# Streampunk/phaneron

Measured on AMD Instinct MI355X. Metric: frames/sec, 4-layer 2160p50 composite pipeline (v210 unpack->CSC->combine->CSC->v210 pack), higher is better.
Workload: dtype f32

## Files before the change

phaneron_amd/csrc/ph_kernels_lds.hip:

```cpp
#include "ph_device.h"
#include "ph_kernels.h"
#include "ph_ldslut.h"

#include <atomic>
#include <cstdlib>

#include <type_traits>

#pragma clang fp contract(off)

#ifndef PH_PROBE
#define PH_PROBE 0
#endif
#if PH_PROBE
constexpr int kProbeWords = 16;
__device__ unsigned long long g_fused_probe[2048 * kProbeWords];
extern "C" int ph_debug_fused_probe(unsigned long long *out, int n_words) {
  return (int)hipMemcpyFromSymbol(out, HIP_SYMBOL(g_fused_probe), (size_t)n_words * 8);
}
#define PH_STAMP_ENTRY() \
  const unsigned long long ph_entry_cycles = __builtin_amdgcn_s_memtime(), ph_entry_ticks = __builtin_amdgcn_s_memrealtime()
#define PH_STAMP(k) PH_STAMP_IF(k, tile_begin == wg_begin)
#define PH_STAMP_IF(k, first_tile)                                                   \
  do {                                                                               \
    if (threadIdx.x == 0 && (first_tile)) {                                          \
      g_fused_probe[blockIdx.x * kProbeWords + 2 * (k)] = __builtin_amdgcn_s_memtime();       \
      g_fused_probe[blockIdx.x * kProbeWords + 2 * (k) + 1] = __builtin_amdgcn_s_memrealtime(); \
      if ((k) == 0) {                                                                \
        g_fused_probe[blockIdx.x * kProbeWords + 10] = ph_entry_cycles;              \
        g_fused_probe[blockIdx.x * kProbeWords + 11] = ph_entry_ticks;               \
      }                                                                              \
    }                                                                                \
  } while (0)
#else
#define PH_STAMP_ENTRY() do { } while (0)
#define PH_STAMP(k) do { } while (0)
#define PH_STAMP_IF(k, first_tile) do { } while (0)
#endif

#ifndef PH_BALANCE_WAVES
#define PH_BALANCE_WAVES 1
#endif
#if PH_BALANCE_WAVES
__device__ __forceinline__ void ph_set_wave_priority(int level) {
  switch (level) {
    case 3: __builtin_amdgcn_s_setprio(3); break;
    case 2: __builtin_amdgcn_s_setprio(2); break;
    case 1: __builtin_amdgcn_s_setprio(1); break;
    default: __builtin_amdgcn_s_setprio(0); break;
  }
}
#define PH_BALANCE(p) ph_set_wave_priority(3 - ((p) * 4) / P)
#else
#define PH_BALANCE(p) do { } while (0)
#endif

namespace ph {


__device__ __forceinline__ uint4 write_quad_lds(const float (&rgb)[18], const WriteK &wk, const LutK &lut) {
  uint32_t y[6], u[3], v[3];
#pragma unroll
  for (int j = 0; j < 6; ++j) {
    if ((j & 1) == 0) {
      const Yuv1 c = write_px_lds(rgb[3 * j], rgb[3 * j + 1], rgb[3 * j + 2], wk, lut);
      y[j] = c.y, u[j >> 1] = c.u, v[j >> 1] = c.v;
    } else {
      y[j] = write_px_luma_lds(rgb[3 * j], rgb[3 * j + 1], rgb[3 * j + 2], wk, lut);
    }
  }
  return pack_quad(y, u, v);
}

#ifndef PH_FUSED_SPLIT
#define PH_FUSED_SPLIT 0
#endif
typedef uint32_t fused_head_line __attribute__((ext_vector_type(16)));
struct FusedHead {
  fused_head_line l0, l1, l2;
  __device__ __forceinline__ uint32_t word(int byte) const { return byte < 64 ? l0[byte / 4] : byte < 128 ? l1[byte / 4 - 16] : l2[byte / 4 - 32]; }
  template <typename P>
  __device__ __forceinline__ P ptr(int byte) const { return (P)((uintptr_t)word(byte) | ((uintptr_t)word(byte + 4) << 32)); }
  __device__ __forceinline__ LutK lut_k(int byte) const {
    return LutK{__uint_as_float(word(byte)), __uint_as_float(word(byte + 4)), __uint_as_float(word(byte + 8)), __uint_as_float(word(byte + 12)), word(byte + 16)};
  }
};
typedef const __attribute__((address_space(1))) ph_u4v *global_quad_ptr;
typedef const __attribute__((address_space(1))) uint32_t *global_u32_ptr;
typedef const __attribute__((address_space(4))) float *const_f32_ptr;
__device__ __forceinline__ uint4 load_stream(global_quad_ptr p) {
  const ph_u4v v = __builtin_nontemporal_load(p);
  return make_uint4(v.x, v.y, v.z, v.w);
}
__device__ __forceinline__ ReadK load_read_k(const_f32_ptr cm, const_f32_ptr gm) {
  ReadK k;
  k.r = make_float4(cm[0], cm[1], cm[2], cm[3]);
  k.g = make_float4(cm[4], cm[5], cm[6], cm[7]);
  k.b = make_float4(cm[8], cm[9], cm[10], cm[11]);
#pragma unroll
  for (int i = 0; i < 9; ++i) k.gm[i] = gm[i];
  return k;
}
__device__ __forceinline__ WriteK load_write_k(const_f32_ptr cm) {
  WriteK k;
  k.y = make_float4(cm[0], cm[1], cm[2], cm[3]);
  k.u = make_float4(cm[4], cm[5], cm[6], cm[7]);
  k.v = make_float4(cm[8], cm[9], cm[10], cm[11]);
  return k;
}
static_assert(kFusedHeadBytes == 3 * sizeof(fused_head_line), "fused_head_load asks for three lines");
__device__ __forceinline__ FusedHead fused_head_load() {
  FusedHead h;
  const auto *args = __builtin_amdgcn_kernarg_segment_ptr();
  asm volatile("s_load_dwordx16 %0, %3, 0x0\n\ts_load_dwordx16 %1, %3, 0x40\n\ts_load_dwordx16 %2, %3, 0x80\n\ts_waitcnt lgkmcnt(0)"
               : "=&s"(h.l0), "=&s"(h.l1), "=&s"(h.l2)
               : "s"(args));
  return h;
}

template <int N, int P, int BS, bool PIPE = false, int MODE = 0, bool TAIL = false>
__global__ __launch_bounds__(BS) void fused_v210_combine_lds_kernel(FusedLdsArgs a, uint32_t *handoff = nullptr) {
  static_assert(!TAIL || (!PIPE && MODE == 0), "the tail instantiation exists for the shipped form only");
  PH_STAMP_ENTRY();
  const FusedHead head = fused_head_load();
  const uint32_t total_quads = head.word(offsetof(FusedLdsArgs, total_quads)), wg_per_job = head.word(offsetof(FusedLdsArgs, wg_per_job));
  const uint32_t per_wg = head.word(offsetof(FusedLdsArgs, per_wg));
  uint32_t job = fused_job_of(blockIdx.x, head.word(offsetof(FusedLdsArgs, magic_wg)));
  asm("" : "+s"(job));
  const uint32_t wg_in_job = blockIdx.x - job * wg_per_job;
  auto layer_ptr = [&](int l) { return reinterpret_cast<const uint4 *>(job ? a.more_layers[job - 1][l] : a.layers[l]); };
  const uint32_t wg_begin = wg_in_job * per_wg;
  const uint32_t wg_end = wg_begin + per_wg < total_quads ? wg_begin + per_wg : total_quads;
  if (wg_begin >= wg_end) return;
  const uint32_t tile_quads = BS * P;
  auto quad_at = [&](uint32_t tile_begin, int p) {
    const uint32_t f = tile_begin + p * BS + threadIdx.x;
    return f < wg_end ? f : wg_end - 1;
  };
  uint4 w;
  if (job) w = load_stream(layer_ptr(0) + quad_at(wg_begin, 0));
  else w = load_stream(head.ptr<global_quad_ptr>(offsetof(FusedLdsArgs, layers)) + quad_at(wg_begin, 0));
  const uint32_t *const rd_blob = (const uint32_t *)head.ptr<global_u32_ptr>(offsetof(FusedLdsArgs, rd_blob));
  const uint32_t rd_bytes = head.word(offsetof(FusedLdsArgs, rd_bytes)), rd_hole = head.word(offsetof(FusedLdsArgs, rd_hole));
  PH_STAMP_IF(0, true);
  if (MODE != 2) lds_lut_load<BS, false>(rd_blob, rd_bytes, rd_hole);
  __builtin_amdgcn_sched_barrier(0);
  const ReadK rk = load_read_k(head.ptr<const_f32_ptr>(offsetof(FusedLdsArgs, rd_cm)), head.ptr<const_f32_ptr>(offsetof(FusedLdsArgs, rd_gm)));
  const WriteK wk = load_write_k(head.ptr<const_f32_ptr>(offsetof(FusedLdsArgs, wr_cm)));
  LutK rlut = head.lut_k(offsetof(FusedLdsArgs, rd_k)), wlut = head.lut_k(offsetof(FusedLdsArgs, wr_k));
  asm("" : "+v"(rlut.a_base), "+v"(rlut.delta_base), "+v"(wlut.a_base), "+v"(wlut.delta_base));
  const uint32_t *const wr_blob = (const uint32_t *)head.ptr<global_u32_ptr>(offsetof(FusedLdsArgs, wr_blob));
  const uint32_t wr_bytes = head.word(offsetof(FusedLdsArgs, wr_bytes)), wr_hole = head.word(offsetof(FusedLdsArgs, wr_hole));
  uint4 *const out_ptr = reinterpret_cast<uint4 *>(job ? a.more_out[job - 1] : a.out);
  const bool std_matrix = ycbcr_matrix_is_standard(rk);
  for (uint32_t tile_begin = wg_begin; tile_begin < wg_end; tile_begin += tile_quads) {
    uint32_t st[P][9];
    auto quad_of = [&](int p) { return quad_at(tile_begin, p); };
    if (tile_begin != wg_begin) {
      w = load_stream(layer_ptr(0) + quad_of(0));
      if (MODE == 0) lds_lut_load<BS, false>(rd_blob, rd_bytes, rd_hole);
    }
    auto slot_kind = [&](uint32_t f) -> uint32_t {
      const uint32_t g = f - __umulhi(f, a.magic_qpp) * a.quads_per_line_pitch;
      return g < a.quads_per_line_used ? 0u : (g == a.quads_per_line_used && a.tail_px) ? 1u : 2u;
    };
    auto phase1_slice = [&](auto tag, uint4 w, uint32_t f, uint32_t f_next, bool more, uint32_t(&st)[9]) -> uint4 {
      const bool in_tail = TAIL && slot_kind(f) == 1u;
      const float last = TAIL ? (in_tail ? 0.0f : 1.0f) : 1.0f;
      float acc[18];
#pragma unroll
      for (int i = 0; i < 18; ++i) acc[i] = 0.0f;
#pragma unroll 1
      for (int l = 0; l < N; ++l) {
        uint4 nxt = w;
        if (l + 1 < N) nxt = load_stream(layer_ptr(l + 1) + f);
        else if (more) nxt = load_stream(layer_ptr(0) + f_next);
        const Yuv6 q = unpack_quad(w);
#pragma unroll
        for (int j = 0; j < 6; ++j) {
          const float4 t = read_px_lds<decltype(tag)::value>(q.y[j], q.cb[j >> 1], q.cr[j >> 1], rk, rlut, last);
          const float kk = 1.0f - t.w;
          asm volatile("v_fma_f32 %0, %0, %3, %4\n\tv_fma_f32 %1, %1, %3, %5\n\tv_fma_f32 %2, %2, %3, %6"
                       : "+v"(acc[3 * j]), "+v"(acc[3 * j + 1]), "+v"(acc[3 * j + 2])
                       : "v"(kk), "v"(t.x), "v"(t.y), "v"(t.z));
        }
        w = nxt;
      }
#pragma unroll
      for (int i = 0; i < 9; ++i) {
        const uint32_t lo = __float_as_uint(TAIL ? lds_lut_index_unit_tail(acc[2 * i], in_tail) : lds_lut_index_unit(acc[2 * i]));
        const uint32_t hi = __float_as_uint(TAIL ? lds_lut_index_unit_tail(acc[2 * i + 1], in_tail) : lds_lut_index_unit(acc[2 * i + 1]));
        st[i] = __builtin_amdgcn_perm(hi, lo, 0x05040100u);
        asm volatile("" : "+v"(st[i]));
      }
      return w;
    };
    if (MODE == 0 || (MODE == 1 && tile_begin == wg_begin)) {
      asm volatile("s_waitcnt vmcnt(0)" ::: "memory");
      __syncthreads();
    }
    PH_STAMP(1);
    const uint32_t tile_left = wg_end - tile_begin;
    if constexpr (PIPE) {
      auto phase1_all = [&](auto tag) {
        constexpr bool STD = decltype(tag)::value;
        auto issue_first = [&](const uint4 &word) {
          return read_px_issue<STD>((float)((word.x >> 10) & 0x3ff), (float)(word.x & 0x3ff), (float)((word.x >> 20) & 0x3ff), rk, rlut);
        };
        auto issue_px = [&](const uint4 &word, int j) {
          const uint32_t wy = j == 0 ? word.x : j < 3 ? word.y : j == 3 ? word.z : word.w;
          const uint32_t sy = (j == 0 || j == 3) ? 10u : (j == 1 || j == 4) ? 0u : 20u;
          const int pr = j >> 1;
          const uint32_t wcb = pr == 0 ? word.x : pr == 1 ? word.y : word.z, scb = 10u * pr;
          const uint32_t wcr = pr == 0 ? word.x : pr == 1 ? word.z : word.w, scr = pr == 0 ? 20u : pr == 1 ? 0u : 10u;
          return read_px_issue<STD>((float)((wy >> sy) & 0x3ff), (float)((wcb >> scb) & 0x3ff), (float)((wcr >> scr) & 0x3ff), rk, rlut);
        };
        PxPending pend = issue_first(w);
#pragma unroll
        for (int p = 0; p < P; ++p) {
          if (p * BS < tile_left) {
            PH_BALANCE(p);
            const uint32_t f = quad_of(p);
            const bool more = (p + 1 < P) && ((p + 1) * BS < tile_left);
            const uint32_t f_next = more ? quad_of(p + 1) : f;
            float acc[18];
#pragma unroll
            for (int i = 0; i < 18; ++i) acc[i] = 0.0f;
#pragma unroll 1
            for (int l = 0; l < N; ++l) {
              uint4 nxt = w;
              if (l + 1 < N) nxt = load_stream(layer_ptr(l + 1) + f);
              else if (more) nxt = load_stream(layer_ptr(0) + f_next);
#pragma unroll
              for (int j = 0; j < 6; ++j) {
                PxPending nx;
                if (j < 5) nx = issue_px(w, j + 1);
                else {
                  uint4 first = nxt;
                  asm volatile("" : "+v"(first.x));
                  nx = issue_first(first);
                }
                __builtin_amdgcn_sched_barrier(0);
                const float4 t = read_px_finish(pend, rk);
                const float kk = 1.0f - t.w;
                asm volatile("v_fma_f32 %0, %0, %3, %4\n\tv_fma_f32 %1, %1, %3, %5\n\tv_fma_f32 %2, %2, %3, %6"
                             : "+v"(acc[3 * j]), "+v"(acc[3 * j + 1]), "+v"(acc[3 * j + 2])
                             : "v"(kk), "v"(t.x), "v"(t.y), "v"(t.z));
                __builtin_amdgcn_sched_barrier(0);
                pend = nx;
              }
              w = nxt;
            }
#pragma unroll
            for (int i = 0; i < 9; ++i) {
              const uint32_t lo = __float_as_uint(lds_lut_index_unit(acc[2 * i]));
              const uint32_t hi = __float_as_uint(lds_lut_index_unit(acc[2 * i + 1]));
              st[p][i] = __builtin_amdgcn_perm(hi, lo, 0x05040100u);
              asm volatile("" : "+v"(st[p][i]));
            }
          }
        }
      };
      if (std_matrix) phase1_all(std::true_type{});
      else phase1_all(std::false_type{});
      PH_STAMP(2);
      __syncthreads();
      lds_lut_load<BS>(wr_blob, wr_bytes, wr_hole);
      __syncthreads();
      PH_STAMP(3);
      auto idx_at = [&](int p, int i) {
        const uint32_t v = st[p][i >> 1];
        return __uint_as_float(((i & 1) ? (v >> 16) : (v & 0xFFFFu)) | 0x4B400000u);
      };
      PxPending wp = write_px_issue(idx_at(0, 0), idx_at(0, 1), idx_at(0, 2), wlut);
#pragma unroll
      for (int p = 0; p < P; ++p) {
        if (p * BS < tile_left) {
          PH_BALANCE(p);
          const uint32_t f = tile_begin + p * BS + threadIdx.x;
          uint32_t y[6], u[3], v[3];
#pragma unroll
          for (int j = 0; j < 6; ++j) {
            PxPending nx = wp;
            if (j < 5) nx = write_px_issue(idx_at(p, 3 * j + 3), idx_at(p, 3 * j + 4), idx_at(p, 3 * j + 5), wlut);
            else if (p + 1 < P) {
              if ((p + 1) * BS < tile_left) nx = write_px_issue(idx_at(p + 1 < P ? p + 1 : p, 0), idx_at(p + 1 < P ? p + 1 : p, 1), idx_at(p + 1 < P ? p + 1 : p, 2), wlut);
            }
            __builtin_amdgcn_sched_barrier(0);
            const float gr = lds_lut_finish(wp.r), gg = lds_lut_finish(wp.g), gb = lds_lut_finish(wp.b);
            y[j] = sat_u16_rte(dot4(gr, gg, gb, 1.0f, wk.y));
            if ((j & 1) == 0) {
              u[j >> 1] = sat_u16_rte(dot4(gr, gg, gb, 1.0f, wk.u));
              v[j >> 1] = sat_u16_rte(dot4(gr, gg, gb, 1.0f, wk.v));
            }
            __builtin_amdgcn_sched_barrier(0);
            wp = nx;
          }
          if (f < wg_end) store_stream(out_ptr + f, pack_quad(y, u, v));
        }
      }
    } else {
    const uint32_t wave_first = (uint32_t)__builtin_amdgcn_readfirstlane((int)(threadIdx.x & ~63u));
    if (MODE != 2) {
#pragma unroll
    for (int p = 0; p < P; ++p) {
      const uint32_t f = quad_of(p);
      if (p * BS + wave_first < wg_end - tile_begin) {
        PH_BALANCE(p);
        const bool more = (p + 1 < P) && ((p + 1) * BS + wave_first < wg_end - tile_begin);
        const uint32_t f_next = more ? quad_of(p + 1) : f;
        if (std_matrix) w = phase1_slice(std::true_type{}, w, f, f_next, more, st[p]);
        else w = phase1_slice(std::false_type{}, w, f, f_next, more, st[p]);
      }
    }
    }
    if (MODE == 1) {
#pragma unroll
      for (int p = 0; p < P; ++p)
        if (p * BS + wave_first < wg_end - tile_begin) {
          const uint32_t f = quad_of(p);
#pragma unroll
          for (int i = 0; i < 9; ++i) handoff[(size_t)i * a.total_quads + f] = st[p][i];
        }
      continue;
    }
    if (MODE == 2) {
#pragma unroll
      for (int p = 0; p < P; ++p)
        if (p * BS + wave_first < wg_end - tile_begin) {
          const uint32_t f = quad_of(p);
#pragma unroll
          for (int i = 0; i < 9; ++i) st[p][i] = __builtin_nontemporal_load(handoff + (size_t)i * a.total_quads + f);
        }
    }
    PH_STAMP(2);
    if (MODE == 0 || tile_begin == wg_begin) {
      __syncthreads();
      lds_lut_load<BS>(wr_blob, wr_bytes, wr_hole);
      __syncthreads();
    }
    PH_STAMP(3);
#pragma unroll
    for (int p = 0; p < P; ++p) {
      const uint32_t f = tile_begin + p * BS + threadIdx.x;
      if (p * BS + wave_first < wg_end - tile_begin) {
        PH_BALANCE(p);
        float yi[18];
#pragma unroll
        for (int i = 0; i < 9; ++i) {
          yi[2 * i] = __uint_as_float((st[p][i] & 0xFFFFu) | 0x4B400000u);
          yi[2 * i + 1] = __uint_as_float((st[p][i] >> 16) | 0x4B400000u);
        }
        uint4 packed;
        if (TAIL) {
          const uint32_t kind = slot_kind(f < wg_end ? f : wg_end - 1);
          if (kind == 0u) packed = write_quad_idx_lds(yi, wk, wlut);
          else if (kind == 1u) packed = write_quad_idx_lds_tail(yi, wk, wlut, a.tail_px);
          else packed = make_uint4(0u, 0u, 0u, 0u);
        } else {
          packed = write_quad_idx_lds(yi, wk, wlut);
        }
        if (f < wg_end) store_stream(out_ptr + f, packed);
      }
    }
    }
    PH_STAMP(4);
    if (PIPE || MODE != 0 || tile_begin + tile_quads < wg_end) __syncthreads();
    PH_STAMP(6);
  }
}

__global__ __launch_bounds__(kLdsBlock) void v210_read_lds_kernel(const uint4 *__restrict__ in, float4 *__restrict__ out,
                                                                   uint32_t width, uint32_t quads_per_line_pitch,
                                                                   uint32_t total_px, const float *__restrict__ cm,
                                                                   const float *__restrict__ gm, LutView lut, uint32_t nt) {
  const ReadK k = load_read_k(cm, gm);
  const LutK lk = make_lut_k(lut);
  lds_lut_load(lut);
  __syncthreads();
  const uint32_t tail_from = width - width % 6u;
  for (uint32_t p = blockIdx.x * kLdsBlock + threadIdx.x; p < total_px; p += gridDim.x * kLdsBlock) {
    const uint32_t line = p / width, x = p - line * width;
    const uint32_t g = x / 6, j = x - 6 * g, pr = j >> 1;
    const uint4 w = in[(size_t)line * quads_per_line_pitch + g];
    const uint32_t wy = (j == 0) ? w.x : (j < 3) ? w.y : (j == 3) ? w.z : w.w;
    const uint32_t sy = (j == 0 || j == 3) ? 10u : (j == 1 || j == 4) ? 0u : 20u;
    const uint32_t wcb = pr == 0 ? w.x : pr == 1 ? w.y : w.z;
    const uint32_t wcr = pr == 0 ? w.x : pr == 1 ? w.z : w.w;
    const uint32_t scr = pr == 0 ? 20u : pr == 1 ? 0u : 10u;
    const float yf = (float)((wy >> sy) & 0x3ff);
    const float cbf = (float)((wcb >> (10u * pr)) & 0x3ff);
    const float crf = (float)((wcr >> scr) & 0x3ff);
    store_image(out + p, read_px_lds(yf, cbf, crf, k, lk, x < tail_from ? 1.0f : 0.0f), nt);
  }
}

struct ReadBatchArgs {
  const uint4 *in[kMaxLayers];
  float4 *out[kMaxLayers];
  uint32_t wg_per_frame;
};
__global__ __launch_bounds__(kLdsBlock) void v210_read_lds_batch_kernel(ReadBatchArgs a, uint32_t width, uint32_t quads_per_line_pitch,
                                                                         uint32_t total_px, const float *__restrict__ cm,
                                                                         const float *__restrict__ gm, LutView lut, uint32_t nt) {
  const ReadK k = load_read_k(cm, gm);
  const LutK lk = make_lut_k(lut);
  lds_lut_load(lut);
  __syncthreads();
  const uint32_t frame = blockIdx.x / a.wg_per_frame, wg = blockIdx.x - frame * a.wg_per_frame;
  const uint4 *__restrict__ in = a.in[frame];
  float4 *__restrict__ out = a.out[frame];
  const uint32_t tail_from = width - width % 6u;
  for (uint32_t p = wg * kLdsBlock + threadIdx.x; p < total_px; p += a.wg_per_frame * kLdsBlock) {
    const uint32_t line = p / width, x = p - line * width;
    const uint32_t g = x / 6, j = x - 6 * g, pr = j >> 1;
    const uint4 w = in[(size_t)line * quads_per_line_pitch + g];
    const uint32_t wy = (j == 0) ? w.x : (j < 3) ? w.y : (j == 3) ? w.z : w.w;
    const uint32_t sy = (j == 0 || j == 3) ? 10u : (j == 1 || j == 4) ? 0u : 20u;
    const uint32_t wcb = pr == 0 ? w.x : pr == 1 ? w.y : w.z;
    const uint32_t wcr = pr == 0 ? w.x : pr == 1 ? w.z : w.w;
    const uint32_t scr = pr == 0 ? 20u : pr == 1 ? 0u : 10u;
    const float yf = (float)((wy >> sy) & 0x3ff);
    const float cbf = (float)((wcb >> (10u * pr)) & 0x3ff);
    const float crf = (float)((wcr >> scr) & 0x3ff);
    store_image(out + p, read_px_lds(yf, cbf, crf, k, lk, x < tail_from ? 1.0f : 0.0f), nt);
  }
}

__global__ __launch_bounds__(kLdsBlock) void v210_write_lds_kernel(const float4 *__restrict__ in, uint4 *__restrict__ out,
                                                                    uint32_t width, uint32_t quads_per_line,
                                                                    uint32_t lines, uint32_t first_line,
                                                                    uint32_t line_step, const float *__restrict__ cm,
                                                                    LutView lut) {
  const WriteK k = load_write_k(cm);
  const LutK lk = make_lut_k(lut);
  lds_lut_load(lut);
  __syncthreads();
  const uint32_t total = quads_per_line * lines, full = width / 6u, remain = width - 6u * full;
  for (uint32_t f = blockIdx.x * kLdsBlock + threadIdx.x; f < total; f += gridDim.x * kLdsBlock) {
    const uint32_t li = f / quads_per_line, g = f - li * quads_per_line;
    const uint32_t line = first_line + li * line_step;
    if (g > full || (g == full && !remain)) {
      store_stream(out + (size_t)line * quads_per_line + g, make_uint4(0u, 0u, 0u, 0u));
      continue;
    }
    const float4 *row = in + (size_t)line * width;
    float rgb[18];
#pragma unroll
    for (int j = 0; j < 6; ++j) {
      const uint32_t x = 6u * g + (uint32_t)j < width ? 6u * g + (uint32_t)j : width - 1u;
      const float4 p = row[x];
      rgb[3 * j] = p.x, rgb[3 * j + 1] = p.y, rgb[3 * j + 2] = p.z;
    }
    if (g == full) {
      float yi[18];
#pragma unroll
      for (int i = 0; i < 18; ++i) yi[i] = lds_lut_index_unit_tail(rgb[i], true);
      store_stream(out + (size_t)line * quads_per_line + g, write_quad_idx_lds_tail(yi, k, lk, remain));
      continue;
    }
    store_stream(out + (size_t)line * quads_per_line + g, write_quad_lds(rgb, k, lk));
  }
}

__global__ __launch_bounds__(kLdsBlock) void compose_write_v210_kernel(ComposeArgs a) {
  const WriteK wk = load_write_k(a.wr_cm);
  const LutK lk = make_lut_k(a.wr);
  lds_lut_load(a.wr);
  __syncthreads();
  const uint32_t qpl = (a.out_w + 47u) / 48u * 8u, full = a.out_w / 6u, remain = a.out_w - 6u * full;
  const uint32_t total = qpl * a.lines;
  for (uint32_t f = blockIdx.x * kLdsBlock + threadIdx.x; f < total; f += gridDim.x * kLdsBlock) {
    const uint32_t li = f / qpl, g = f - li * qpl;
    const uint32_t line = a.first_line + li * a.line_step;
    if (g > full || (g == full && !remain)) {
      store_stream(reinterpret_cast<uint4 *>(a.out) + (size_t)line * qpl + g, make_uint4(0u, 0u, 0u, 0u));
      continue;
    }
    float acc[24];
#pragma unroll 1
    for (int l = 0; l < a.n; ++l) {
      const float4 *img = reinterpret_cast<const float4 *>(a.layers[l]);
      const int lw = a.lw[l], lh = a.lh[l];
      const float *m = a.matrix[l];
      float m0 = 0, m1 = 0, m2 = 0, m3 = 0, m4 = 0, m5 = 0;
      if (m) m0 = m[0], m1 = m[1], m2 = m[2], m3 = m[3], m4 = m[4], m5 = m[5];
      const float py = (float)(int)line / (float)(int)a.out_h - 0.5f;
#pragma unroll
      for (int j = 0; j < 6; ++j) {
        const int x = 6 * g + j < a.out_w ? (int)(6 * g + j) : (int)a.out_w - 1;
        float4 t;
        if (m) {
          const float px = (float)x / (float)(int)a.out_w - 0.5f;
          const float s = dot3(m0, m1, m2, px, py, 1.0f) + 0.5f;
          const float tt = dot3(m3, m4, m5, px, py, 1.0f) + 0.5f;
          t = sample_linear(img, lw, lh, s, tt);
        } else {
          t = img[(size_t)line * a.out_w + x];
        }
        if (l == 0) {
          acc[4 * j] = t.x, acc[4 * j + 1] = t.y, acc[4 * j + 2] = t.z, acc[4 * j + 3] = t.w;
        } else {
          const float kk = 1.0f - t.w;
          acc[4 * j] = fma_rn(acc[4 * j], kk, t.x);
          acc[4 * j + 1] = fma_rn(acc[4 * j + 1], kk, t.y);
          acc[4 * j + 2] = fma_rn(acc[4 * j + 2], kk, t.z);
          acc[4 * j + 3] = fma_rn(acc[4 * j + 3], 0.0f, t.w);
        }
      }
    }
    float rgb[18];
#pragma unroll
    for (int j = 0; j < 6; ++j) rgb[3 * j] = acc[4 * j], rgb[3 * j + 1] = acc[4 * j + 1], rgb[3 * j + 2] = acc[4 * j + 2];
    if (g == full) {
      float yi[18];
#pragma unroll
      for (int i = 0; i < 18; ++i) yi[i] = lds_lut_index_unit_tail(rgb[i], true);
      store_stream(reinterpret_cast<uint4 *>(a.out) + (size_t)line * qpl + g, write_quad_idx_lds_tail(yi, wk, lk, remain));
      continue;
    }
    store_stream(reinterpret_cast<uint4 *>(a.out) + (size_t)line * qpl + g, write_quad_lds(rgb, wk, lk));
  }
}

constexpr uint32_t kComposeChunk = 192;
constexpr uint32_t kComposeStageBytes = (kLdsBlock / 64) * kComposeChunk * 4;
template <int N, bool ALL_DIRECT>
__global__ __launch_bounds__(kLdsBlock) void compose_write_v210_px_kernel(ComposeArgs a, uint32_t stage_off) {
  const WriteK wk = load_write_k(a.wr_cm);
  const LutK lk = make_lut_k(a.wr);
  float mm[N][6];
  bool direct[N];
#pragma unroll
  for (int l = 0; l < N; ++l) {
    direct[l] = a.matrix[l] == nullptr;
#pragma unroll
    for (int i = 0; i < 6; ++i) mm[l][i] = direct[l] ? 0.0f : a.matrix[l][i];
  }
  lds_lut_load(a.wr);
  __syncthreads();
  const uint32_t wave = threadIdx.x >> 6, lane = threadIdx.x & 63;
  uint16_t *ys = reinterpret_cast<uint16_t *>(g_lds + stage_off + wave * kComposeChunk * 4);
  uint16_t *us = ys + kComposeChunk, *vs = us + kComposeChunk / 2;
  const uint32_t qpl = a.out_w / 6;
  const uint32_t total_px = a.out_w * a.lines;
  const uint32_t waves_total = gridDim.x * (kLdsBlock / 64);
  for (uint32_t base = (blockIdx.x * (kLdsBlock / 64) + wave) * kComposeChunk; base < total_px;
       base += waves_total * kComposeChunk) {
#pragma unroll 1
    for (uint32_t k = 0; k < kComposeChunk / 64; ++k) {
      const uint32_t local = k * 64 + lane;
      uint32_t p = base + local;
      p = p < total_px ? p : total_px - 1;
      const uint32_t li = p / a.out_w, x = p - li * a.out_w;
      const uint32_t line = a.first_line + li * a.line_step;
      const float py = (float)(int)line / (float)(int)a.out_h - 0.5f;
      const float px = (float)(int)x / (float)(int)a.out_w - 0.5f;
      float4 t[N];
#pragma unroll
      for (int l = 0; l < N; ++l) {
        if (ALL_DIRECT) {
          t[l] = load_stream(reinterpret_cast<const float4 *>(a.layers[l]) + (size_t)line * a.out_w + x);
          continue;
        }
        const float s = dot3(mm[l][0], mm[l][1], mm[l][2], px, py, 1.0f) + 0.5f;
        const float tt = dot3(mm[l][3], mm[l][4], mm[l][5], px, py, 1.0f) + 0.5f;
        t[l] = sample_linear<true>(reinterpret_cast<const float4 *>(a.layers[l]), a.lw[l], a.lh[l], s, tt, direct[l], x, line);
      }
      float r = t[0].x, g = t[0].y, b = t[0].z;
#pragma unroll
      for (int l = 1; l < N; ++l) {
        const float kk = 1.0f - t[l].w;
        r = fma_rn(r, kk, t[l].x), g = fma_rn(g, kk, t[l].y), b = fma_rn(b, kk, t[l].z);
      }
      const Yuv1 c = write_px_lds(r, g, b, wk, lk);
      ys[local] = (uint16_t)c.y;
      if (!(x & 1)) us[local >> 1] = (uint16_t)c.u, vs[local >> 1] = (uint16_t)c.v;
    }
    __builtin_amdgcn_fence(__ATOMIC_RELEASE, "wavefront");
    __builtin_amdgcn_wave_barrier();
    __builtin_amdgcn_fence(__ATOMIC_ACQUIRE, "wavefront");
    if (lane < kComposeChunk / 6) {
      const uint32_t first_px = base + lane * 6;
      if (first_px < total_px) {
        uint32_t y[6], u[3], v[3];
#pragma unroll
        for (int j = 0; j < 6; ++j) y[j] = ys[lane * 6 + j];
#pragma unroll
        for (int j = 0; j < 3; ++j) u[j] = us[lane * 3 + j], v[j] = vs[lane * 3 + j];
        const uint32_t li = first_px / a.out_w, x = first_px - li * a.out_w;
        const uint32_t line = a.first_line + li * a.line_step;
        store_stream(reinterpret_cast<uint4 *>(a.out) + (size_t)line * qpl + x / 6, pack_quad(y, u, v));
      }
    }
    __builtin_amdgcn_wave_barrier();
  }
}

#ifndef PH_COMPOSE_GROUP_ROWS
#define PH_COMPOSE_GROUP_ROWS 16
#endif
typedef uint32_t ph_u32x4 __attribute__((ext_vector_type(4)));
constexpr uint32_t kTapOutside = 0x80000000u;

struct RowTaps {
  uint32_t r0, r1;
// ... 72 lines not shown
      }
      uint32_t o00 = 0, o10 = 0, o01 = 0, o11 = 0;
#pragma unroll
      for (int l = 0; l < N; ++l) {
        if (SHARED && l > 0) {
          wa[l] = wa[0], wb[l] = wb[0];
          tap[l][0] = __builtin_amdgcn_raw_buffer_load_b128(img[l], (int)o00, 0, 0);
          tap[l][1] = __builtin_amdgcn_raw_buffer_load_b128(img[l], (int)o10, 0, 0);
          tap[l][2] = __builtin_amdgcn_raw_buffer_load_b128(img[l], (int)o01, 0, 0);
          tap[l][3] = __builtin_amdgcn_raw_buffer_load_b128(img[l], (int)o11, 0, 0);
          continue;
        }
        const RowTaps r = ALIGNED ? row[l] : row_taps(dot3(mm[l][3], mm[l][4], mm[l][5], px, py, 1.0f) + 0.5f, a.lw[l], a.lh[l]);
        const float s = dot3(mm[l][0], mm[l][1], mm[l][2], px, py, 1.0f) + 0.5f;
        const float u = s * (float)a.lw[l];
        const float fu = u - 0.5f;
        const float flu = __builtin_floorf(fu);
        const uint32_t i0 = (uint32_t)(int)flu, i1 = i0 + 1u;
        const uint32_t c0 = i0 < (uint32_t)a.lw[l] ? i0 << 4 : kTapOutside, c1 = i1 < (uint32_t)a.lw[l] ? i1 << 4 : kTapOutside;
        wa[l] = fu - flu, wb[l] = r.b;
        o00 = r.r0 + c0, o10 = r.r0 + c1, o01 = r.r1 + c0, o11 = r.r1 + c1;
        if (MIXED) o00 = direct[l] ? own : o00;
        tap[l][0] = __builtin_amdgcn_raw_buffer_load_b128(img[l], (int)o00, 0, 0);
#ifdef PH_TAPS_ONE_LOAD
        tap[l][1] = tap[l][0] + o10, tap[l][2] = tap[l][0] + o01, tap[l][3] = tap[l][0] + o11;
#else
        tap[l][1] = __builtin_amdgcn_raw_buffer_load_b128(img[l], (int)o10, 0, 0);
        tap[l][2] = __builtin_amdgcn_raw_buffer_load_b128(img[l], (int)o01, 0, 0);
        tap[l][3] = __builtin_amdgcn_raw_buffer_load_b128(img[l], (int)o11, 0, 0);
#endif
      }
      float r = 0.0f, g = 0.0f, b = 0.0f;
#pragma unroll
      for (int l = 0; l < N; ++l) {
        const float4 t00 = as_float4(tap[l][0]), t10 = as_float4(tap[l][1]), t01 = as_float4(tap[l][2]), t11 = as_float4(tap[l][3]);
        const float oma = 1.0f - wa[l], omb = 1.0f - wb[l];
        const float w00 = oma * omb, w10 = wa[l] * omb, w01 = oma * wb[l], w11 = wa[l] * wb[l];
        float4 t;
        t.x = ((w00 * t00.x + w10 * t10.x) + w01 * t01.x) + w11 * t11.x;
        t.y = ((w00 * t00.y + w10 * t10.y) + w01 * t01.y) + w11 * t11.y;
        t.z = ((w00 * t00.z + w10 * t10.z) + w01 * t01.z) + w11 * t11.z;
        t.w = ((w00 * t00.w + w10 * t10.w) + w01 * t01.w) + w11 * t11.w;
        if (MIXED) t.x = direct[l] ? t00.x : t.x, t.y = direct[l] ? t00.y : t.y, t.z = direct[l] ? t00.z : t.z, t.w = direct[l] ? t00.w : t.w;
        if (WIPE && a.wipe_with[l]) {
          const float m = wipe_m[l], rm = 1.0f - m;
          t.x = fma_rn(wipe_b[l].x, m, t.x * rm), t.y = fma_rn(wipe_b[l].y, m, t.y * rm);
          t.z = fma_rn(wipe_b[l].z, m, t.z * rm), t.w = fma_rn(wipe_b[l].w, m, t.w * rm);
        }
        if (l == 0) {
          r = t.x, g = t.y, b = t.z;
        } else {
          const float kk = 1.0f - t.w;
          r = fma_rn(r, kk, t.x), g = fma_rn(g, kk, t.y), b = fma_rn(b, kk, t.z);
        }
      }
      const Yuv1 c = write_px_lds(r, g, b, wk, lk);
      ys[local] = (uint16_t)c.y;
      if (!(x & 1)) us[local >> 1] = (uint16_t)c.u, vs[local >> 1] = (uint16_t)c.v;
    }
    __builtin_amdgcn_fence(__ATOMIC_RELEASE, "wavefront");
    __builtin_amdgcn_wave_barrier();
    __builtin_amdgcn_fence(__ATOMIC_ACQUIRE, "wavefront");
    if (lane < kComposeChunk / 6) {
      uint32_t y[6], u[3], v[3];
#pragma unroll
      for (int j = 0; j < 6; ++j) y[j] = ys[lane * 6 + j];
#pragma unroll
      for (int j = 0; j < 3; ++j) u[j] = us[lane * 3 + j], v[j] = vs[lane * 3 + j];
      store_stream(reinterpret_cast<uint4 *>(a.out) + (size_t)line * qpl + (x_first + lane * 6) / 6, pack_quad(y, u, v));
    }
    __builtin_amdgcn_wave_barrier();
  }
}

template <int N, bool MIXED, bool SHARED = false, bool WIPE = false>
__global__ __launch_bounds__(kLdsBlock) void compose_write_v210_taps_kernel(ComposeArgs a, uint32_t stage_off) {
  const WriteK wk = load_write_k(a.wr_cm);
  const LutK lk = make_lut_k(a.wr);
  float mm[N][6];
  bool direct[N];
  __amdgpu_buffer_rsrc_t img[N];
  bool all_aligned = true;
#pragma unroll
  for (int l = 0; l < N; ++l) {
    direct[l] = a.matrix[l] == nullptr;
#pragma unroll
    for (int i = 0; i < 6; ++i) mm[l][i] = direct[l] ? 0.0f : a.matrix[l][i];
    all_aligned = all_aligned && mm[l][1] == 0.0f && mm[l][3] == 0.0f;
    img[l] = __builtin_amdgcn_make_buffer_rsrc(const_cast<void *>(a.layers[l]), 0, a.lw[l] * a.lh[l] * 16, 0x00020000);
  }
  lds_lut_load(a.wr);
  __syncthreads();
  const uint32_t wave = __builtin_amdgcn_readfirstlane(threadIdx.x >> 6), lane = threadIdx.x & 63;
  uint16_t *ys = reinterpret_cast<uint16_t *>(g_lds + stage_off + wave * kComposeChunk * 4);
  uint16_t *us = ys + kComposeChunk, *vs = us + kComposeChunk / 2;
  if (all_aligned)
    compose_taps_body<N, MIXED, true, SHARED, WIPE>(a, mm, direct, img, wk, lk, ys, us, vs, wave, lane);
  else
    compose_taps_body<N, MIXED, false, SHARED, WIPE>(a, mm, direct, img, wk, lk, ys, us, vs, wave, lane);
}

template <int N>
static hipError_t launch_compose_taps_n(hipStream_t s, const ComposeArgs &a, uint32_t grid, uint32_t stage_off) {
  bool mixed = false, shared = N > 1, wipe = false;
  for (int l = 0; l < N; ++l) {
    wipe = wipe || a.wipe_with[l] != nullptr;
    mixed = mixed || a.matrix[l] == nullptr;
    shared = shared && a.matrix[l] != nullptr && a.matrix[l] == a.matrix[0] && a.lw[l] == a.lw[0] && a.lh[l] == a.lh[0];
  }
  if (wipe) {
    hipError_t e = hipFuncSetAttribute(reinterpret_cast<const void *>(compose_write_v210_taps_kernel<N, true, false, true>),
                                       hipFuncAttributeMaxDynamicSharedMemorySize, kMaxDynamicLds);
    if (e != hipSuccess) return e;
    compose_write_v210_taps_kernel<N, true, false, true><<<grid, kLdsBlock, stage_off + kComposeStageBytes, s>>>(a, stage_off);
    return hipGetLastError();
  }
  const void *fn = shared ? reinterpret_cast<const void *>(compose_write_v210_taps_kernel<N, false, true>)
                   : mixed ? reinterpret_cast<const void *>(compose_write_v210_taps_kernel<N, true>)
                           : reinterpret_cast<const void *>(compose_write_v210_taps_kernel<N, false>);
  hipError_t e = hipFuncSetAttribute(fn, hipFuncAttributeMaxDynamicSharedMemorySize, kMaxDynamicLds);
  if (e != hipSuccess) return e;
  if (shared)
    compose_write_v210_taps_kernel<N, false, true><<<grid, kLdsBlock, stage_off + kComposeStageBytes, s>>>(a, stage_off);
  else if (mixed)
    compose_write_v210_taps_kernel<N, true><<<grid, kLdsBlock, stage_off + kComposeStageBytes, s>>>(a, stage_off);
  else
    compose_write_v210_taps_kernel<N, false><<<grid, kLdsBlock, stage_off + kComposeStageBytes, s>>>(a, stage_off);
  return hipGetLastError();
}

static bool compose_taps_eligible(const ComposeArgs &a) {
  if (a.out_w % kComposeChunk) return false;
  bool sampled = false;
  for (int l = 0; l < a.n; ++l) {
    const uint64_t bytes = (uint64_t)a.lw[l] * (uint64_t)a.lh[l] * 16u, pitch = (uint64_t)a.lw[l] * 16u;
    if (bytes + 2 * pitch > 0x80000000ull || pitch >= (1u << 23) || a.lh[l] >= (1 << 22)) return false;
    sampled = sampled || a.matrix[l] != nullptr;
  }
  for (int l = 0; l < a.n; ++l) sampled = sampled || a.wipe_with[l] != nullptr;
  return sampled;
}
static bool compose_stage_fits(const ComposeArgs &a) { return ((a.wr.bytes + 15u) & ~15u) + kComposeStageBytes <= 160u * 1024u; }
static bool compose_quad_forced() {
  static const int quad_env = [] {
    const char *e = getenv("PH_COMPOSE_QUAD");
    return e ? atoi(e) : 0;
  }();
  return quad_env != 0;
}
static bool compose_taps_enabled() {
  static const int taps_env = [] {
    const char *e = getenv("PH_COMPOSE_TAPS");
    return e ? atoi(e) : 1;
  }();
  return taps_env != 0;
}
static bool compose_uses_taps(const ComposeArgs &a) {
  return !compose_quad_forced() && compose_stage_fits(a) && compose_taps_enabled() && compose_taps_eligible(a);
}
bool compose_can_wipe(const ComposeArgs &a) { return compose_uses_taps(a); }

template <int N, bool ALL_DIRECT>
static hipError_t launch_compose_px_nd(hipStream_t s, const ComposeArgs &a, uint32_t grid, uint32_t stage_off) {
  hipError_t e = hipFuncSetAttribute(reinterpret_cast<const void *>(compose_write_v210_px_kernel<N, ALL_DIRECT>),
                                     hipFuncAttributeMaxDynamicSharedMemorySize, kMaxDynamicLds);
  if (e != hipSuccess) return e;
  compose_write_v210_px_kernel<N, ALL_DIRECT><<<grid, kLdsBlock, stage_off + kComposeStageBytes, s>>>(a, stage_off);
  return hipGetLastError();
}
template <int N>
static hipError_t launch_compose_px_n(hipStream_t s, const ComposeArgs &a, uint32_t grid, uint32_t stage_off) {
  bool all_direct = true;
  for (int l = 0; l < N; ++l) all_direct = all_direct && a.matrix[l] == nullptr;
  return all_direct ? launch_compose_px_nd<N, true>(s, a, grid, stage_off) : launch_compose_px_nd<N, false>(s, a, grid, stage_off);
}

template <typename K>
static hipError_t allow_lds(K kernel, uint32_t bytes) {
  return hipFuncSetAttribute(reinterpret_cast<const void *>(kernel), hipFuncAttributeMaxDynamicSharedMemorySize, kMaxDynamicLds);
}
template <typename K>
static hipError_t allow_lds_once(K kernel, std::atomic<uint64_t> &done) {
  int dev = 0;
  hipError_t e = hipGetDevice(&dev);
  if (e != hipSuccess) return e;
  const uint64_t bit = 1ull << (dev & 63);
  if (dev < 64 && (done.load(std::memory_order_acquire) & bit)) return hipSuccess;
  e = allow_lds(kernel, kMaxDynamicLds);
  if (e == hipSuccess && dev < 64) done.fetch_or(bit, std::memory_order_release);
  return e;
}

FusedLutK fused_lut_k(const LutView &v) {
#if defined(__x86_64__)
  const unsigned csr = __builtin_ia32_stmxcsr();
  __builtin_ia32_ldmxcsr(csr & ~0x8040u);
#endif
  const volatile float lds0 = 0.0f, magic = 12582912.0f;
  const float small = (v.delta_base + lds0) + v.bias * v.delta_scale;
  const float b = small - magic * v.delta_scale;
  const FusedLutK k{v.a_scale, -((magic - v.bias) * v.a_scale), v.delta_scale, b, v.shift - 2u};
#if defined(__x86_64__)
  __builtin_ia32_ldmxcsr(csr);
#endif
  return k;
}

FusedLdsArgs fused_lds_args(const FusedArgs &f, const LutView &rd, const LutView &wr) {
  FusedLdsArgs a{};
  a.rd_blob = rd.blob, a.rd_bytes = rd.bytes, a.rd_hole = rd.hole;
  a.wr_blob = wr.blob, a.wr_bytes = wr.bytes, a.wr_hole = wr.hole;
  a.rd_k = fused_lut_k(rd), a.wr_k = fused_lut_k(wr);
  for (int l = 0; l < kMaxLayers; ++l) a.layers[l] = f.layers[l];
  a.out = f.out, a.rd_cm = f.rd_cm, a.rd_gm = f.rd_gm, a.wr_cm = f.wr_cm;
  a.total_quads = f.total_quads, a.quads_per_line_used = f.quads_per_line_used, a.quads_per_line_pitch = f.quads_per_line_pitch;
  a.tail_px = f.tail_px, a.magic_qpp = f.magic_qpp, a.jobs = 1;
  return a;
}

#if PH_FUSED_SPLIT
template <int N, int P, int BS, int MODE>
static hipError_t launch_fused_half(hipStream_t s, FusedLdsArgs b, uint32_t lds) {
  static uint32_t *handoff = nullptr;
  static size_t handoff_quads = 0;
  if (handoff_quads < b.total_quads) {
    if (handoff) hipFree(handoff);
    if (hipMalloc(&handoff, (size_t)b.total_quads * 36) != hipSuccess) return hipErrorOutOfMemory;
    handoff_quads = b.total_quads;
  }
  static std::atomic<uint64_t> lds_allowed{0};
  hipError_t e = allow_lds_once(fused_v210_combine_lds_kernel<N, P, BS, false, MODE>, lds_allowed);
  if (e != hipSuccess) return e;
  fused_v210_combine_lds_kernel<N, P, BS, false, MODE><<<b.wg_per_job * b.jobs, BS, lds, s>>>(b, handoff);
  return hipGetLastError();
}
#endif

template <int N, int P, int BS, bool PIPE = false, bool TAIL = false>
static hipError_t launch_fused_npb(hipStream_t s, const FusedLdsArgs &a, uint32_t grid_in, uint32_t lds) {
  uint32_t grid = grid_in;
#if PH_FUSED_SPLIT
  static const int cus_env = [] {
    const char *e = getenv("PH_FUSED_CUS");
    return e ? atoi(e) : 0;
  }();
  if (cus_env > 0 && (uint32_t)cus_env < grid) grid = (uint32_t)cus_env;
#endif
  static std::atomic<uint64_t> lds_allowed{0};
  hipError_t e = allow_lds_once(fused_v210_combine_lds_kernel<N, P, BS, PIPE, 0, TAIL>, lds_allowed);
  if (e != hipSuccess) return e;
  const uint32_t slices = (a.total_quads + BS - 1) / BS;
  FusedLdsArgs b = a;
  if (b.jobs < 1) b.jobs = 1;
  b.wg_per_job = grid / b.jobs ? grid / b.jobs : 1;
  if (b.wg_per_job > slices) b.wg_per_job = slices;
  b.per_wg = (b.total_quads + b.wg_per_job - 1) / b.wg_per_job;
  b.magic_wg = fused_wg_magic(b.wg_per_job);
#if PH_FUSED_SPLIT
  if (!PIPE && N == 4) {
    static const int mode_env = [] {
      const char *e = getenv("PH_FUSED_MODE");
      return e ? atoi(e) : 0;
    }();
    if (mode_env == 1) return launch_fused_half<N, P, BS, 1>(s, b, lds);
    if (mode_env == 2) return launch_fused_half<N, P, BS, 2>(s, b, lds);
    if (mode_env == 3) {
      hipError_t e1 = launch_fused_half<N, P, BS, 1>(s, b, lds);
      return e1 != hipSuccess ? e1 : launch_fused_half<N, P, BS, 2>(s, b, lds);
    }
  }
#endif
  fused_v210_combine_lds_kernel<N, P, BS, PIPE, 0, TAIL><<<b.wg_per_job * b.jobs, BS, lds, s>>>(b);
  return hipGetLastError();
}

template <int N>
static hipError_t launch_fused_n(hipStream_t s, const FusedLdsArgs &a, uint32_t grid, uint32_t lds) {
  static const int geom_env = [] {
    const char *e = getenv("PH_FUSED_GEOM");
    return e ? atoi(e) : 0;
  }();
  if (a.quads_per_line_used != a.quads_per_line_pitch) return launch_fused_npb<N, 6, 1024, false, true>(s, a, grid, lds);
  int geom = geom_env ? geom_env : 6;
  static const int pipe_env = [] {
    const char *e = getenv("PH_FUSED_PIPE");
    return e ? atoi(e) : 0;
  }();
#ifdef PH_FUSED_EXPERIMENT
  static const int bs_env = [] {
    const char *e = getenv("PH_FUSED_BS");
    return e ? atoi(e) : 0;
  }();
  if (N == 4 && bs_env == 768) return pipe_env ? launch_fused_npb<4, 8, 768, true>(s, a, grid, lds) : launch_fused_npb<4, 8, 768>(s, a, grid, lds);
  if (N == 4 && bs_env == 512) return pipe_env ? launch_fused_npb<4, 11, 512, true>(s, a, grid, lds) : launch_fused_npb<4, 11, 512>(s, a, grid, lds);
#endif
  if (pipe_env && geom == 6) return launch_fused_npb<N, 6, 1024, true>(s, a, grid, lds);
  if (geom == 4) return launch_fused_npb<N, 4, 1024>(s, a, grid, lds);
  if (geom == 8) return launch_fused_npb<N, 8, 1024>(s, a, grid, lds);
  return launch_fused_npb<N, 6, 1024>(s, a, grid, lds);
}

hipError_t launch_fused_v210_combine_lds(hipStream_t s, int n, const FusedLdsArgs &a, uint32_t num_cus) {
  const uint32_t lds = a.rd_bytes > a.wr_bytes ? a.rd_bytes : a.wr_bytes;
  switch (n) {
    case 1: return launch_fused_n<1>(s, a, num_cus, lds);
    case 2: return launch_fused_n<2>(s, a, num_cus, lds);
    case 3: return launch_fused_n<3>(s, a, num_cus, lds);
    case 4: return launch_fused_n<4>(s, a, num_cus, lds);
    case 5: return launch_fused_n<5>(s, a, num_cus, lds);
    case 6: return launch_fused_n<6>(s, a, num_cus, lds);
    case 7: return launch_fused_n<7>(s, a, num_cus, lds);
    case 8: return launch_fused_n<8>(s, a, num_cus, lds);
    default: return hipErrorInvalidValue;
  }
}

hipError_t launch_compose_write_v210(hipStream_t s, const ComposeArgs &a, uint32_t num_cus) {
  const uint32_t total = (a.out_w + 47u) / 48u * 8u * a.lines;
  if (!total) return hipSuccess;
  bool any_wipe = false;
  for (int l = 0; l < a.n; ++l) any_wipe = any_wipe || a.wipe_with[l] != nullptr;
  if (any_wipe && !compose_uses_taps(a)) return hipErrorInvalidValue;
  const uint32_t stage_off = (a.wr.bytes + 15u) & ~15u;
  if (!compose_quad_forced() && compose_stage_fits(a) && a.out_w % 48u == 0) {
    const uint32_t chunks = (a.out_w * a.lines + kComposeChunk - 1) / kComposeChunk;
    const uint32_t want = (chunks + kLdsBlock / 64 - 1) / (kLdsBlock / 64);
    const uint32_t grid = want < num_cus ? want : num_cus;
    if (compose_uses_taps(a)) {
      switch (a.n) {
        case 1: return launch_compose_taps_n<1>(s, a, grid, stage_off);
        case 2: return launch_compose_taps_n<2>(s, a, grid, stage_off);
        case 3: return launch_compose_taps_n<3>(s, a, grid, stage_off);
        case 4: return launch_compose_taps_n<4>(s, a, grid, stage_off);
        case 5: return launch_compose_taps_n<5>(s, a, grid, stage_off);
        case 6: return launch_compose_taps_n<6>(s, a, grid, stage_off);
        case 7: return launch_compose_taps_n<7>(s, a, grid, stage_off);
        case 8: return launch_compose_taps_n<8>(s, a, grid, stage_off);
        default: return hipErrorInvalidValue;
      }
    }
    switch (a.n) {
      case 1: return launch_compose_px_n<1>(s, a, grid, stage_off);
      case 2: return launch_compose_px_n<2>(s, a, grid, stage_off);
      case 3: return launch_compose_px_n<3>(s, a, grid, stage_off);
      case 4: return launch_compose_px_n<4>(s, a, grid, stage_off);
      case 5: return launch_compose_px_n<5>(s, a, grid, stage_off);
      case 6: return launch_compose_px_n<6>(s, a, grid, stage_off);
      case 7: return launch_compose_px_n<7>(s, a, grid, stage_off);
      case 8: return launch_compose_px_n<8>(s, a, grid, stage_off);
      default: return hipErrorInvalidValue;
    }
  }
  hipError_t e = allow_lds(compose_write_v210_kernel, a.wr.bytes);
  if (e != hipSuccess) return e;
  const uint32_t want = (total + kLdsBlock - 1) / kLdsBlock;
  compose_write_v210_kernel<<<want < num_cus ? want : num_cus, kLdsBlock, a.wr.bytes, s>>>(a);
  return hipGetLastError();
}

__global__ void lds_base_probe_kernel(uint32_t *out) {
  *out = (uint32_t)(uintptr_t)(__attribute__((address_space(3))) unsigned char *)g_lds;
}
hipError_t launch_lds_base_probe(hipStream_t s, uint32_t *out_dev) {
  lds_base_probe_kernel<<<1, 64, 16, s>>>(out_dev);
  return hipGetLastError();
}

hipError_t launch_v210_read_lds(hipStream_t s, const void *in, void *out, uint32_t width, uint32_t height,
                                const void *cm, const void *gm, const LutView &lut, uint32_t num_cus) {
  hipError_t e = allow_lds(v210_read_lds_kernel, lut.bytes);
  if (e != hipSuccess) return e;
  const uint32_t total = width * height;
  const uint32_t want = (total + kLdsBlock - 1) / kLdsBlock;
  v210_read_lds_kernel<<<want < num_cus ? want : num_cus, kLdsBlock, lut.bytes, s>>>(
      (const uint4 *)in, (float4 *)out, width, v210_pitch_bytes(width) / 16, total, (const float *)cm, (const float *)gm,
      lut, image_nt((size_t)width * height * 16));
  return hipGetLastError();
}

hipError_t launch_v210_read_lds_batch(hipStream_t s, int n, const void *const *ins, void *const *outs, uint32_t width,
                                      uint32_t height, const void *cm, const void *gm, const LutView &lut, uint32_t num_cus) {
  hipError_t e = allow_lds(v210_read_lds_batch_kernel, lut.bytes);
  if (e != hipSuccess) return e;
  ReadBatchArgs a{};
  for (int i = 0; i < n; ++i) a.in[i] = (const uint4 *)ins[i], a.out[i] = (float4 *)outs[i];
  const uint32_t total = width * height;
  const uint32_t want = (total + kLdsBlock - 1) / kLdsBlock;
  uint32_t per = num_cus / (uint32_t)n ? num_cus / (uint32_t)n : 1;
  a.wg_per_frame = want < per ? want : per;
  v210_read_lds_batch_kernel<<<a.wg_per_frame * n, kLdsBlock, lut.bytes, s>>>(a, width, v210_pitch_bytes(width) / 16, total,
                                                                              (const float *)cm, (const float *)gm, lut,
                                                                              image_nt((size_t)width * height * 16));
  return hipGetLastError();
}

hipError_t launch_v210_write_lds(hipStream_t s, const void *in, void *out, uint32_t width, uint32_t height,
                                 uint32_t interlace, const void *cm, const LutView &lut, uint32_t num_cus) {
  hipError_t e = allow_lds(v210_write_lds_kernel, lut.bytes);
  if (e != hipSuccess) return e;
  const uint32_t step = interlace ? 2 : 1, first = (interlace == 3) ? 1 : 0;
  const uint32_t lines = interlace ? height / 2 : height, qpl = v210_pitch_bytes(width) / 16;
  if (!lines) return hipSuccess;
  const uint32_t want = (qpl * lines + kLdsBlock - 1) / kLdsBlock;
  v210_write_lds_kernel<<<want < num_cus ? want : num_cus, kLdsBlock, lut.bytes, s>>>(
      (const float4 *)in, (uint4 *)out, width, qpl, lines, first, step, (const float *)cm, lut);
  return hipGetLastError();
}

}
```

Before: 20340.

## Unroll layer combine loop with peeled first/last layers and scalar layer pointers

Replaces the runtime per-layer loop in phase 1 with a compile-time structure. The first layer initialises the accumulator directly, middle layers use plain FMAs, and the last layer uses FMA with hardware clamp so the separate clamp before the LUT index is skipped. Layer base pointers are kept in the scalar kernarg head, patched per job, and addressed with byte offsets, which removes per-iteration pointer selection. In exchange the code grows larger and may need more registers, and a guard now rejects total_quads above 2^28 so the byte offsets stay within 32 bits.

```diff
diff --git a/phaneron_amd/csrc/ph_kernels_lds.hip b/phaneron_amd/csrc/ph_kernels_lds.hip
--- a/phaneron_amd/csrc/ph_kernels_lds.hip
+++ b/phaneron_amd/csrc/ph_kernels_lds.hip
@@ -6,6 +6,7 @@
 #include <cstdlib>
 
 #include <type_traits>
+#include <utility>
 
 #pragma clang fp contract(off)
 
@@ -79,6 +80,11 @@
 struct FusedHead {
   fused_head_line l0, l1, l2;
   __device__ __forceinline__ uint32_t word(int byte) const { return byte < 64 ? l0[byte / 4] : byte < 128 ? l1[byte / 4 - 16] : l2[byte / 4 - 32]; }
+  __device__ __forceinline__ void set_word(int byte, uint32_t v) {
+    if (byte < 64) l0[byte / 4] = v;
+    else if (byte < 128) l1[byte / 4 - 16] = v;
+    else l2[byte / 4 - 32] = v;
+  }
   template <typename P>
   __device__ __forceinline__ P ptr(int byte) const { return (P)((uintptr_t)word(byte) | ((uintptr_t)word(byte + 4) << 32)); }
   __device__ __forceinline__ LutK lut_k(int byte) const {
@@ -118,11 +124,53 @@
   return h;
 }
 
+constexpr int kLayerFirst = 1, kLayerLast = 2;
+template <int... I, typename F>
+__device__ __forceinline__ void static_for_each(std::integer_sequence<int, I...>, F &&f) {
+  (f(std::integral_constant<int, I>{}), ...);
+}
+template <int COUNT, typename F>
+__device__ __forceinline__ void static_for(F &&f) {
+  static_for_each(std::make_integer_sequence<int, COUNT>{}, f);
+}
+template <int PLACE, bool STD>
+__device__ __forceinline__ void fused_layer_combine(float (&acc)[18], const uint4 w, const ReadK &rk, const LutK &rlut, float last) {
+  __builtin_amdgcn_sched_barrier(0);
+  const Yuv6 q = unpack_quad(w);
+#pragma unroll
+  for (int j = 0; j < 6; ++j) {
+    const float4 t = read_px_lds<STD>(q.y[j], q.cb[j >> 1], q.cr[j >> 1], rk, rlut, last);
+    if (PLACE & kLayerFirst) {
+      acc[3 * j] = t.x, acc[3 * j + 1] = t.y, acc[3 * j + 2] = t.z;
+      if (PLACE & kLayerLast) {
+#pragma unroll
+        for (int c = 0; c < 3; ++c) acc[3 * j + c] = __builtin_fminf(__builtin_fmaxf(acc[3 * j + c], 0.0f), 1.0f);
+      }
+      asm volatile("" : "+v"(acc[3 * j]), "+v"(acc[3 * j + 1]), "+v"(acc[3 * j + 2]));
+    } else {
+      const float kk = 1.0f - t.w;
+      if (PLACE & kLayerLast)
+        asm volatile("v_fma_f32 %0, %0, %3, %4 clamp\n\tv_fma_f32 %1, %1, %3, %5 clamp\n\tv_fma_f32 %2, %2, %3, %6 clamp"
+                     : "+v"(acc[3 * j]), "+v"(acc[3 * j + 1]), "+v"(acc[3 * j + 2])
+                     : "v"(kk), "v"(t.x), "v"(t.y), "v"(t.z));
+      else
+        asm volatile("v_fma_f32 %0, %0, %3, %4\n\tv_fma_f32 %1, %1, %3, %5\n\tv_fma_f32 %2, %2, %3, %6"
+                     : "+v"(acc[3 * j]), "+v"(acc[3 * j + 1]), "+v"(acc[3 * j + 2])
+                     : "v"(kk), "v"(t.x), "v"(t.y), "v"(t.z));
+    }
+  }
+}
+__device__ __forceinline__ float lds_lut_index_clamped(float t) { return t * 65535.0f + kRoundMagic; }
+__device__ __forceinline__ float lds_lut_index_clamped_tail(float t, bool trunc) {
+  const float x = t * 65535.0f;
+  return (trunc ? __builtin_floorf(x) : x) + kRoundMagic;
+}
+
 template <int N, int P, int BS, bool PIPE = false, int MODE = 0, bool TAIL = false>
 __global__ __launch_bounds__(BS) void fused_v210_combine_lds_kernel(FusedLdsArgs a, uint32_t *handoff = nullptr) {
   static_assert(!TAIL || (!PIPE && MODE == 0), "the tail instantiation exists for the shipped form only");
   PH_STAMP_ENTRY();
-  const FusedHead head = fused_head_load();
+  FusedHead head = fused_head_load();
   const uint32_t total_quads = head.word(offsetof(FusedLdsArgs, total_quads)), wg_per_job = head.word(offsetof(FusedLdsArgs, wg_per_job));
   const uint32_t per_wg = head.word(offsetof(FusedLdsArgs, per_wg));
   uint32_t job = fused_job_of(blockIdx.x, head.word(offsetof(FusedLdsArgs, magic_wg)));
@@ -137,8 +185,38 @@
     const uint32_t f = tile_begin + p * BS + threadIdx.x;
     return f < wg_end ? f : wg_end - 1;
   };
+  constexpr bool kSplitLayers = !PIPE && MODE == 0;
+  if (kSplitLayers && job) {
+    auto own_layer = [&](int l) {
+      const uintptr_t p = (uintptr_t)a.more_layers[job - 1][l];
+      head.set_word(offsetof(FusedLdsArgs, layers) + 8 * l, (uint32_t)p);
+      head.set_word(offsetof(FusedLdsArgs, layers) + 8 * l + 4, (uint32_t)(p >> 32));
+    };
+    own_layer(0);
+    if (N > 1) own_layer(1);
+    if (N > 2) own_layer(2);
+    if (N > 3) own_layer(3);
+    if (N > 4) own_layer(4);
+    if (N > 5) own_layer(5);
+    if (N > 6) own_layer(6);
+    if (N > 7) own_layer(7);
+  }
+  static_assert(N <= 8, "the layers' pointers are named one by one");
+  typedef const __attribute__((address_space(1))) char *global_byte_ptr;
+  auto layer_base = [&](int l) { return (global_byte_ptr)head.ptr<global_quad_ptr>(offsetof(FusedLdsArgs, layers) + 8 * l); };
+  auto layer_word = [&](int l, uint32_t at) { return load_stream((global_quad_ptr)(layer_base(l) + at)); };
+  auto layer_word_any = [&](int l, uint32_t at) {
+    global_byte_ptr base = layer_base(N - 1);
+    if (N > 3 && l == 2) base = layer_base(2);
+    if (N > 4 && l == 3) base = layer_base(3);
+    if (N > 5 && l == 4) base = layer_base(4);
+    if (N > 6 && l == 5) base = layer_base(5);
+    if (N > 7 && l == 6) base = layer_base(6);
+    return load_stream((global_quad_ptr)(base + at));
+  };
   uint4 w;
-  if (job) w = load_stream(layer_ptr(0) + quad_at(wg_begin, 0));
+  if (kSplitLayers) w = layer_word(0, quad_at(wg_begin, 0) << 4);
+  else if (job) w = load_stream(layer_ptr(0) + quad_at(wg_begin, 0));
   else w = load_stream(head.ptr<global_quad_ptr>(offsetof(FusedLdsArgs, layers)) + quad_at(wg_begin, 0));
   const uint32_t *const rd_blob = (const uint32_t *)head.ptr<global_u32_ptr>(offsetof(FusedLdsArgs, rd_blob));
   const uint32_t rd_bytes = head.word(offsetof(FusedLdsArgs, rd_bytes)), rd_hole = head.word(offsetof(FusedLdsArgs, rd_hole));
@@ -157,7 +235,7 @@
     uint32_t st[P][9];
     auto quad_of = [&](int p) { return quad_at(tile_begin, p); };
     if (tile_begin != wg_begin) {
-      w = load_stream(layer_ptr(0) + quad_of(0));
+      w = kSplitLayers ? layer_word(0, quad_of(0) << 4) : load_stream(layer_ptr(0) + quad_of(0));
       if (MODE == 0) lds_lut_load<BS, false>(rd_blob, rd_bytes, rd_hole);
     }
     auto slot_kind = [&](uint32_t f) -> uint32_t {
@@ -190,6 +268,64 @@
       for (int i = 0; i < 9; ++i) {
         const uint32_t lo = __float_as_uint(TAIL ? lds_lut_index_unit_tail(acc[2 * i], in_tail) : lds_lut_index_unit(acc[2 * i]));
         const uint32_t hi = __float_as_uint(TAIL ? lds_lut_index_unit_tail(acc[2 * i + 1], in_tail) : lds_lut_index_unit(acc[2 * i + 1]));
+        st[i] = __builtin_amdgcn_perm(hi, lo, 0x05040100u);
+        asm volatile("" : "+v"(st[i]));
+      }
+      return w;
+    };
+    auto phase1_slice_split = [&](auto tag, uint4 w, uint32_t f, uint32_t f_next, bool more, uint32_t(&st)[9]) __attribute__((always_inline)) -> uint4 {
+      constexpr int MID = N > 2 ? N - 2 : 0;
+      const bool in_tail = TAIL && slot_kind(f) == 1u;
+      const float last = TAIL ? (in_tail ? 0.0f : 1.0f) : 1.0f;
+      float acc[18];
+      constexpr bool STD = decltype(tag)::value;
+      auto combine = [&](auto place, const uint4 word) __attribute__((always_inline)) {
+        fused_layer_combine<decltype(place)::value, STD>(acc, word, rk, rlut, last);
+      };
+      constexpr std::integral_constant<int, N == 1 ? (kLayerFirst | kLayerLast) : kLayerFirst> first_layer{};
+      constexpr std::integral_constant<int, 0> middle_layer{};
+      constexpr std::integral_constant<int, kLayerLast> last_layer{};
+      uint32_t at = f << 4;
+      if (STD) asm volatile("; standard matrix" : "+v"(at));
+      else asm volatile("; any matrix" : "+v"(at));
+      uint4 nxt = w;
+      if (N > 1) nxt = layer_word(1, at);
+      else if (more) nxt = layer_word(0, f_next << 4);
+      combine(first_layer, w);
+      w = nxt;
+      if constexpr (MID > 0 && MID <= 2) {
+        nxt = layer_word(2, at);
+        combine(middle_layer, w);
+        w = nxt;
+        if constexpr (MID == 2) {
+          nxt = layer_word(3, at);
+          combine(middle_layer, w);
+          w = nxt;
+        }
+      } else if constexpr (MID > 2) {
+#pragma unroll 1
+        for (int l = 1; l + 1 <= MID; l += 2) {
+          const uint4 w2 = layer_word_any(l + 1, at);
+          combine(middle_layer, w);
+          w = layer_word_any(l + 2, at);
+          combine(middle_layer, w2);
+        }
+        if (MID & 1) {
+          nxt = layer_word(N - 1, at);
+          combine(middle_layer, w);
+          w = nxt;
+        }
+      }
+      if constexpr (N > 1) {
+        nxt = w;
+        if (more) nxt = layer_word(0, f_next << 4);
+        combine(last_layer, w);
+        w = nxt;
+      }
+#pragma unroll
+      for (int i = 0; i < 9; ++i) {
+        const uint32_t lo = __float_as_uint(TAIL ? lds_lut_index_clamped_tail(acc[2 * i], in_tail) : lds_lut_index_clamped(acc[2 * i]));
+        const uint32_t hi = __float_as_uint(TAIL ? lds_lut_index_clamped_tail(acc[2 * i + 1], in_tail) : lds_lut_index_clamped(acc[2 * i + 1]));
         st[i] = __builtin_amdgcn_perm(hi, lo, 0x05040100u);
         asm volatile("" : "+v"(st[i]));
       }
@@ -301,7 +437,19 @@
       }
     } else {
     const uint32_t wave_first = (uint32_t)__builtin_amdgcn_readfirstlane((int)(threadIdx.x & ~63u));
-    if (MODE != 2) {
+    if constexpr (kSplitLayers) {
+      static_for<P>([&](auto slice) __attribute__((always_inline)) {
+        constexpr int p = decltype(slice)::value;
+        const uint32_t f = quad_of(p);
+        if (p * BS + wave_first < wg_end - tile_begin) {
+          PH_BALANCE(p);
+          const bool more = (p + 1 < P) && ((p + 1) * BS + wave_first < wg_end - tile_begin);
+          const uint32_t f_next = more ? quad_of(p + 1) : f;
+          if (std_matrix) w = phase1_slice_split(std::true_type{}, w, f, f_next, more, st[p]);
+          else w = phase1_slice_split(std::false_type{}, w, f, f_next, more, st[p]);
+        }
+      });
+    } else if (MODE != 2) {
 #pragma unroll
     for (int p = 0; p < P; ++p) {
       const uint32_t f = quad_of(p);
@@ -980,6 +1128,7 @@
 
 hipError_t launch_fused_v210_combine_lds(hipStream_t s, int n, const FusedLdsArgs &a, uint32_t num_cus) {
   const uint32_t lds = a.rd_bytes > a.wr_bytes ? a.rd_bytes : a.wr_bytes;
+  if (a.total_quads > (1u << 28)) return hipErrorInvalidValue;
   switch (n) {
     case 1: return launch_fused_n<1>(s, a, num_cus, lds);
     case 2: return launch_fused_n<2>(s, a, num_cus, lds);
```

Result: faster. 20750, median of 6 (+2.0%).
